# Avokadoen/zig_vulkan

Hardware: AMD Instinct MI355X
Metric: Mrays/s at 1920x1080 on 512^3 brickmap (8^3 bricks, primary + shadow, 1 spp); achieved % of HBM roofline (higher is better)
Workload: dtype f32

## Files before the change

### zig_vulkan_amd/csrc/vrt_api.hip

```cpp
#include <hip/hip_runtime.h>
#include <algorithm>
#include <cstdio>
#include <cstdlib>
#include <cstring>
#include <mutex>
#include <new>
#include <string>
#include <thread>
#include "host_brick_grid.hpp"
#include "vrt_ctx.h"

using namespace vrt_impl;

namespace {
thread_local std::string g_create_error;
}

namespace vrt_impl {

int fail(vrt_ctx *ctx, int code, const std::string &msg) {
    if (ctx) ctx->err = msg;
    else g_create_error = msg;
    return code;
}
// ... 492 lines not shown
        p.split_all = (eligible && waves <= 2u * simds) ? 1u : 0u;
#ifdef VRT_EXP_SPLIT_ALL
        if (c->sched.tile_order == 3u) p.split_all = VRT_EXP_SPLIT_ALL;
#endif
    }
    p.brick_batch = (cfg->kernel_variant >> 24) & 0xFu ? ((cfg->kernel_variant >> 24) & 0xFu) * 4u : 8u;
    p.path_brick_batch = (cfg->kernel_variant >> 24) & 0xFu ? ((cfg->kernel_variant >> 24) & 0xFu) * 4u : 32u;
    p.block_threads = ((vrt::resolve_variant(c->cfg.kernel_variant) & 0xFFu) == vrt::kVariantLinearLds512) ? 512u : 256u;
    {
        auto gcd = [](uint32_t a, uint32_t b) { while (b) { const uint32_t t = a % b; a = b; b = t; } return a; };
        uint32_t st = (uint32_t)((double)sh.owned_tiles * 0.6180339887) | 1u;
        while (sh.owned_tiles > 1u && gcd(st, sh.owned_tiles) != 1u) st += 2u;
        p.tile_stride = sh.owned_tiles > 1u ? st % sh.owned_tiles : 0u;
        if (sh.owned_tiles > 1u && p.tile_stride == 0u) p.tile_stride = 1u;
    }
    p.nbx = nbx;
    p.nby = nby;
    p.nbz = nbz;
    if (c->stream_b) {
        VRT_CREATE_HIP(hipEventRecord(c->ev_upload, c->stream));
        c->upload_seq = 1;
    }
#undef VRT_CREATE_HIP
    note_kernel(c, c->product[2] ? c->product[2] : c->kernel_single1);
    *out = c;
    return VRT_OK;
}

void vrt_destroy(vrt_ctx *ctx) { free_ctx(ctx); }

// ... 169 lines not shown
```

### zig_vulkan_amd/csrc/vrt_internal.h

```cpp
#pragma once
#include <hip/hip_runtime.h>
#include <stddef.h>
#include <stdint.h>
#include "../../include/vrt_hip.h"

namespace vrt {

struct PushConstants {
    vrt_camera_device cam;
    vrt_sun_device sun;
};
static_assert(sizeof(vrt_camera_device) == 96, "Camera.Device is 96 bytes (Camera.zig:183-193)");
static_assert(sizeof(vrt_sun_device) == 32, "Sun.Device is 32 bytes (Sun.zig:13-18)");
static_assert(sizeof(PushConstants) == 128, "push constant range is 128 bytes (ComputePipeline.zig:258-272)");
static_assert(sizeof(vrt_grid_state) == 64, "State.Device is 64 bytes (State.zig:60-79)");
static_assert(sizeof(vrt_material) == 20, "Material is 20 bytes (gpu_types.zig:16-32)");

struct DeviceCounters {
    unsigned long long rays, status_loads, bricks_entered, voxel_steps, hits, grid_steps;
    unsigned long long wave_grid_iters, wave_brick_walks, wave_voxel_iters;
};

struct TileOwnership {
    uint32_t period;
// ... 15 lines not shown
    uint32_t skip_to_box;
    const int *cell_bounds;
    uint32_t status_cells, status_words;
    const uint32_t *start_is_slot;
    uint32_t occupancy_words, count_box;
};
struct BrickArgs {
    const uint32_t *cell_box;
    const uint8_t *status_bytes;
    const vrt_material *materials;
    const uint32_t *brick_status, *brick_index;
    const uint8_t *brick_occupancy;
    const uint32_t *brick_start_index;
    const uint8_t *material_index;
};
static_assert(sizeof(TileArgs) == 64 && sizeof(GridExtra) == 48 && sizeof(BrickArgs) == 64, "16, 12 and 16 dwords: s_load_dwordx16, x8 + x4, x16");

struct TraceParams {
    vrt_grid_state grid;
    PushConstants pcs[8];
    const vrt_material *materials;
    const uint32_t *brick_status;
    const uint32_t *brick_index;
    const uint8_t *brick_occupancy;
    const uint32_t *brick_start_index;
    const uint8_t *material_index;
    uint8_t *target_rgba8;
    float *target_rgba32f;
    DeviceCounters *counters;
    uint32_t width, height;
    uint32_t batch_target_stride;
// ... 43 lines not shown
    uint32_t pool_cus;
    float4 *pool_samples;
    uint32_t pool_walk_k;
    uint32_t pool_brick_thr;
    uint32_t pool_trans_thr;
    uint32_t pool_walk_min;
    uint32_t pool_tiles_x_magic;
    uint32_t wave_groups_bounce;
    uint32_t split_all;
    uint32_t count_box;
    uint32_t skip_to_box;
    uint32_t tile_order;
    alignas(16) TileArgs tile_args;
    GridExtra grid_extra;
    BrickArgs brick_args;
};
static_assert(offsetof(TraceParams, grid) == 0 && offsetof(TraceParams, tile_args) % 16 == 0, "the wide scalar loads' offsets");

constexpr int kMaxBatchFrames = 8;
constexpr int kTileW = 16;
constexpr int kTileH = 16;

enum : uint32_t {
    kVariantDefault = 0,
    kVariantLiteral = 1,
    kVariantBlocked = 2,
    kVariantBlockedLds = 3,
    kVariantLinearWide = 4,
    kVariantLinearAlways = 5,
    kVariantLinearLds = 6,
    kVariantLinearLds512 = 7,
    kVariantLinearAhead = 8,
// ... 9 lines not shown
```

### zig_vulkan_amd/csrc/vrt_trace.hip

```cpp
#include <hip/hip_runtime.h>
#include <cstdlib>
#include "vrt_internal.h"
#include "vrt_kernels.h"

namespace vrt {

template <typename PIX>
__global__ __launch_bounds__(256) void vrt_assemble_kernel(const PIX *__restrict__ gathered, PIX *__restrict__ frame, uint32_t width,
                                                           uint32_t height, uint32_t tiles_x, uint32_t shard_count,
                                                           uint32_t tiles_per_rank ,
                                                           const TileOwnership own, uint32_t frame_src_stride ) {
    gathered += (size_t)blockIdx.z * frame_src_stride;
    frame += (size_t)blockIdx.z * width * height;
    const uint32_t x = blockIdx.x * 64u + (threadIdx.x & 63u);
    const uint32_t y = blockIdx.y * 4u + (threadIdx.x >> 6);
    if (x >= width || y >= height) return;
    const uint32_t t = (y / kTileH) * tiles_x + (x / kTileW);
    uint32_t r, i;
    if (own.period) {
        const uint32_t q = t / own.period, j = t % own.period;
        r = own.owner[j];
        i = q * own.count[r] + own.prefix[j];
    } else {
        r = t % shard_count;
// ... 190 lines not shown
static bool is_path_filter_kernel(KernelFn fn) {
    const KernelEntry *e = kernel_entry_of(fn);
    return e && e->path == 1 && e->filter;
}
const char *kernel_name_of(KernelFn fn) {
    const KernelEntry *e = kernel_entry_of(fn);
    return e ? e->name : "?";
}

static void fill_arg_blocks(TraceParams &q) {
    q.tile_args = TileArgs{q.tile_order, q.wave_groups, q.split_all, q.owned_tiles, q.sched_extra, q.own_period, q.tile_schedule, q.wave_timeline,
                           q.own_count, q.shard_rank, q.shard_count, q.tiles_x, q.width, q.height};
    q.grid_extra = GridExtra{q.scale_pow2, q.inv_grid_scale, q.inv_voxel_scale, q.skip_to_box, q.cell_bounds, q.status_cells, q.status_words, q.start_is_slot,
                             q.occupancy_words, q.count_box};
    q.brick_args = BrickArgs{q.cell_box, q.status_bytes, q.materials, q.brick_status, q.brick_index, q.brick_occupancy, q.brick_start_index, q.material_index};
}

hipError_t launch_trace(KernelFn fn, const TraceParams &params, size_t lds_bytes, hipStream_t stream, uint32_t frames) {
    if (params.owned_tiles == 0 || frames == 0) return hipSuccess;
    TraceParams p = params;
    fill_arg_blocks(p);
    if (const KernelEntry *pe = kernel_entry_of(fn); pe && pe->path == 2) {
        if (!p.work_counter || !p.pool_paths || !p.pool_samples || frames != 1u) return hipErrorInvalidValue;
        hipError_t e = hipMemsetAsync(p.work_counter, 0, kMaxBatchFrames * sizeof(uint32_t), stream);
        if (e != hipSuccess) return e;
        const uint64_t units = (uint64_t)p.owned_tiles * 256u * (uint64_t)(p.pcs[0].cam.samples_per_pixel > 0 ? p.pcs[0].cam.samples_per_pixel : 1);
        const uint32_t per_group = 4u * (64u + pe->pool_slots), fit = (uint32_t)std::min<uint64_t>((units + per_group - 1u) / per_group, 1u << 30);
        const uint32_t hold = p.pool_cus * pe->min_waves;
        const uint32_t groups = fit < hold ? (fit ? fit : 1u) : hold;
        VRT_LAUNCH(fn, dim3(groups, 1), dim3(256), pool_group_lds_bytes(pe->pool_slots, pe->pool_stages), stream, p);
// ... 70 lines not shown
```

### zig_vulkan_amd/csrc/vrt_trace_kernels.h

```cpp
#pragma once
#include <hip/hip_runtime.h>
#include "vrt_internal.h"
#include "vrt_kernels.h"
#include "vrt_math.h"

namespace vrt {

constexpr uint32_t MAT_LAMBERTIAN = 0, MAT_METAL = 1, MAT_DIELECTRIC = 2, MAT_NONE = 3;

struct Ray {
    f3 origin, direction;
    float internal_reflection;
    uint32_t ignore_type_material;
};

struct Hit {
    f3 point, normal;
    float t;
    uint32_t index;
};

template <bool COUNT>
struct Cnt {
    uint32_t rays = 0, status_loads = 0, bricks_entered = 0, voxel_steps = 0, hits = 0, grid_steps = 0;
// ... 740 lines not shown
    BrickArgs a;
    uint32_t occupancy_words;
    uint32_t start_is_slot;
    uint32_t scale_pow2;
    float inv_voxel_scale;
};
template <typename T>
VRT_DI T opaque_uniform(T v) {
    asm volatile("" : "+s"(v));
    return v;
}
template <typename T>
VRT_DI const __attribute__((address_space(1))) T *global_ptr(const T *ptr) {
    return (const __attribute__((address_space(1))) T *)ptr;
}
VRT_DI uint32_t scalar_load_u32(const uint32_t *ptr) {
    uint32_t v;
    asm volatile("s_load_dword %0, %1, 0x0\n\ts_waitcnt lgkmcnt(0)" : "=s"(v) : "s"(ptr));
    return v;
}
typedef __attribute__((ext_vector_type(8))) uint32_t u32x8;
typedef __attribute__((ext_vector_type(16))) uint32_t u32x16;
typedef __attribute__((ext_vector_type(2))) uint32_t u32x2;
VRT_DI unsigned long long kernarg_address() { return (unsigned long long)__builtin_amdgcn_kernarg_segment_ptr(); }
struct DerivedPtrs {
    const int *cell_bounds;
    const uint32_t *start_is_slot;
    uint32_t skip_to_box;
};
VRT_DI TileArgs kernarg_tile_args(DerivedPtrs &dp) {
    u32x16 v;
    u32x2 b, f;
    asm volatile("s_load_dwordx16 %0, %4, %5\n\ts_load_dwordx2 %1, %4, %6\n\ts_load_dwordx2 %2, %4, %7\n\ts_load_dword %3, %4, %8\n\ts_waitcnt lgkmcnt(0)"
                 : "=&s"(v), "=&s"(b), "=&s"(f), "=&s"(dp.skip_to_box)
                 : "s"(kernarg_address()), "n"(offsetof(TraceParams, tile_args)), "n"(offsetof(TraceParams, grid_extra) + offsetof(GridExtra, cell_bounds)),
                   "n"(offsetof(TraceParams, grid_extra) + offsetof(GridExtra, start_is_slot)), "n"(offsetof(TraceParams, grid_extra) + offsetof(GridExtra, skip_to_box)));
    dp.cell_bounds = (const int *)__builtin_bit_cast(unsigned long long, b);
    dp.start_is_slot = (const uint32_t *)__builtin_bit_cast(unsigned long long, f);
    return __builtin_bit_cast(TileArgs, v);
}

struct DerivedWords {
    int bounds[6];
    uint32_t start_is_slot;
};
struct EarlyBox {
    DerivedWords dw;
    float g_min[3], g_scale;
    bool test;
};
VRT_DI vrt_camera_device kernarg_camera_box(uint32_t frame, const DerivedPtrs &dp, EarlyBox &eb) {
    struct Parts { u32x16 a; u32x8 b; } v;
    u32x4 lo, gm;
    u32x2 hi;
    uint32_t flag, sc;
    const unsigned long long ka = kernarg_address();
    const unsigned long long at = ka + offsetof(TraceParams, pcs) + (unsigned long long)frame * sizeof(PushConstants);
    const unsigned long long b = dp.cell_bounds ? (unsigned long long)dp.cell_bounds : ka, f = dp.start_is_slot ? (unsigned long long)dp.start_is_slot : ka;
    asm volatile("s_load_dwordx16 %0, %7, 0x0\n\ts_load_dwordx8 %1, %7, 0x40\n\ts_load_dwordx4 %2, %8, 0x0\n\ts_load_dwordx2 %3, %8, 0x10\n\t"
                 "s_load_dword %4, %9, 0x0\n\ts_load_dwordx4 %5, %10, %11\n\ts_load_dword %6, %10, %12\n\ts_waitcnt lgkmcnt(0)"
                 : "=&s"(v.a), "=&s"(v.b), "=&s"(lo), "=&s"(hi), "=&s"(flag), "=&s"(gm), "=&s"(sc)
                 : "s"(at), "s"(b), "s"(f), "s"(ka), "n"(offsetof(TraceParams, grid) + offsetof(vrt_grid_state, min_point_base_t)),
                   "n"(offsetof(TraceParams, grid) + offsetof(vrt_grid_state, max_point_scale) + 12));
    eb.dw = DerivedWords{{(int)lo.x, (int)lo.y, (int)lo.z, (int)lo.w, (int)hi.x, (int)hi.y}, dp.start_is_slot ? flag : 0u};
    const uint32_t gx = gm.x, gy = gm.y, gz = gm.z;
    eb.g_min[0] = __builtin_bit_cast(float, gx), eb.g_min[1] = __builtin_bit_cast(float, gy), eb.g_min[2] = __builtin_bit_cast(float, gz);
    eb.g_scale = __builtin_bit_cast(float, sc);
    eb.test = dp.cell_bounds != nullptr && dp.skip_to_box != 0u;
    struct Padded { vrt_camera_device cam; uint32_t pad[8]; };
    static_assert(sizeof(Parts) == sizeof(Padded) && offsetof(Parts, b) == 64, "x16 | x8, padded to the alignment of the first");
    return __builtin_bit_cast(Padded, v).cam;
}
VRT_DI vrt_sun_device kernarg_sun(uint32_t frame) {
    u32x8 v;
    const unsigned long long at = kernarg_address() + offsetof(TraceParams, pcs) + (unsigned long long)frame * sizeof(PushConstants) + offsetof(PushConstants, sun);
    asm volatile("s_load_dwordx8 %0, %1, 0x0\n\ts_waitcnt lgkmcnt(0)" : "=&s"(v) : "s"(at));
    return __builtin_bit_cast(vrt_sun_device, v);
}
struct GridArgs {
    vrt_grid_state grid;
    uint32_t scale_pow2;
    float inv_grid_scale, inv_voxel_scale;
    uint32_t skip_to_box;
    const int *cell_bounds;
    uint32_t status_cells, status_words;
    const uint32_t *start_is_slot;
    uint32_t occupancy_words, count_box;
};
static_assert(sizeof(GridArgs) == sizeof(vrt_grid_state) + sizeof(GridExtra) && offsetof(GridArgs, cell_bounds) - 64 == offsetof(GridExtra, cell_bounds) &&
                  offsetof(GridArgs, start_is_slot) - 64 == offsetof(GridExtra, start_is_slot) && offsetof(GridArgs, count_box) - 64 == offsetof(GridExtra, count_box),
              "GridArgs = vrt_grid_state + GridExtra, field for field");
// ... 665 lines not shown
    f3 direction = mk3(0, 0, 0);
    const bool should_refract = transmission_direction(ir, r_in.internal_reflection, r_in.direction, normal, direction);
    if (should_refract && rand_3(hit.point) > 0.5f) {
        scattered = create_ray(hit.point, direction);
        scattered.ignore_type_material = MAT_DIELECTRIC;
        scattered.internal_reflection = ir;
    } else {
        direction = reflect3(r_in.direction, normal);
        scattered = create_ray(hit.point, direction);
    }
    return true;
}

template <int B, bool COUNT, int MODE, bool SCALAR_ENTRY = false, bool REJECT = false, bool KARGS = false>
VRT_DI f3 ray_color_single(const TraceParams &p, const PushConstants &pc, const uint32_t *lds_filter, const Ray &ray, Cnt<COUNT> &c,
                           const EarlyBox *eb = nullptr) {
    f3 color = mk3(0, 0, 0);
    int loop_count = 0;
    Hit hit;
    [[maybe_unused]] vrt_sun_device sun_batch;
    bool sun_enabled = false;
    f3 sun_color = mk3(0, 0, 0);
    if constexpr (!KARGS) sun_enabled = pc.sun.enabled > 0, sun_color = mk3(pc.sun.color[0], pc.sun.color[1], pc.sun.color[2]);
    bool primary_hit;
    if constexpr (KARGS) {
        const f3 inv = mk3(safe_inverse(ray.direction.x), safe_inverse(ray.direction.y), safe_inverse(ray.direction.z));
        const bool miss = eb->test && box_miss(ray.origin, inv, eb->dw.bounds, mk3(eb->g_min[0], eb->g_min[1], eb->g_min[2]), eb->g_scale);
        primary_hit = false;
        if (pc.cam.max_bounce > 0 && __builtin_amdgcn_ballot_w64(!miss) != 0ull) {
            primary_hit = grid_hit<B, COUNT, MODE, false, SCALAR_ENTRY, false, REJECT, KARGS>(p, lds_filter, ray, hit, c, nullptr, &eb->dw, miss);
        }
    } else {
        primary_hit = pc.cam.max_bounce > 0 && grid_hit<B, COUNT, MODE, false, SCALAR_ENTRY, false, REJECT, KARGS>(p, lds_filter, ray, hit, c);
    }
    if constexpr (KARGS) {
        sun_batch = kernarg_sun(blockIdx.y);
        sun_enabled = sun_batch.enabled > 0, sun_color = mk3(sun_batch.color[0], sun_batch.color[1], sun_batch.color[2]);
    }
    const vrt_sun_device &sun = KARGS ? sun_batch : pc.sun;
    if (primary_hit) {
        const uint32_t material = hit.index;
        bool lit = true;
        if (sun_enabled) {
            const f3 sun_position = mk3(sun.position[0], sun.position[1], sun.position[2]);
            const f3 rv = rand_vec3_range(ray.direction.x + ray.direction.z, ray.direction.y + ray.direction.z, -sun.radius,
                                          sun.radius);
            const Ray shadow_ray = create_ray(hit.point, (sun_position + rv) - hit.point);
            Hit shadow_hit;
            lit = !grid_hit<B, COUNT, MODE, false, SCALAR_ENTRY, false, REJECT, KARGS>(p, lds_filter, shadow_ray, shadow_hit, c);
        }
        const vrt_material *m = p.materials + material;
        const uint32_t mtype = m->type;
        const f3 attenuation = mk3(m->albedo_r, m->albedo_g, m->albedo_b);
        loop_count = (mtype <= MAT_DIELECTRIC) ? 1 : 0;
        if (sun_enabled) {
// ... 77 lines not shown
    return (xcd < rem) ? xcd * (q + 1u) + i : rem * (q + 1u) + (xcd - rem) * q + i;
}


VRT_DI uint32_t fresh_lane() {
    uint32_t l;
    asm volatile("v_mbcnt_lo_u32_b32 %0, -1, 0\n\tv_mbcnt_hi_u32_b32 %0, -1, %0" : "=v"(l));
    return l;
}

template <int B, bool COUNT, int MODE, int MIN_WAVES, int SHADE, int BLOCK = 256>
__global__ __launch_bounds__(BLOCK, MIN_WAVES) void vrt_trace_kernel(const TraceParams p) {
    extern __shared__ __attribute__((aligned(16))) uint32_t lds_filter[];
    constexpr bool KARGS = SHADE == 2 && !COUNT && BLOCK == 256 && (MODE == kStatusLinearAlways || MODE == kStatusBytes);
    [[maybe_unused]] TileArgs ta;
    [[maybe_unused]] DerivedPtrs dp;
    if constexpr (KARGS) ta = kernarg_tile_args(dp);
#define VRT_TA(field) (KARGS ? ta.field : p.field)
    if constexpr (MODE == kStatusLinearLds) {
        const uint32_t nvec = (p.status_words + 3u) >> 2;
        const uint4 *src = reinterpret_cast<const uint4 *>(p.brick_status);
        uint4 *dst = reinterpret_cast<uint4 *>(lds_filter);
        for (uint32_t i = threadIdx.x; i < nvec; i += blockDim.x) dst[i] = src[i];
        __syncthreads();
    }
    if constexpr (MODE == kStatusBlockedLds) {
        const uint32_t nwords = (p.nbx * p.nby * p.nbz + 31u) >> 5;
        const uint32_t *src = reinterpret_cast<const uint32_t *>(p.status_blocks + (size_t)p.nbx * p.nby * p.nbz);
        for (uint32_t i = threadIdx.x; i < nwords; i += blockDim.x) lds_filter[i] = src[i];
        __syncthreads();
    }
    const uint32_t unit = VRT_TA(wave_groups) ? (blockIdx.x >> 2) : (BLOCK == 512 ? blockIdx.x * 2u + (threadIdx.x >> 8) : (blockIdx.x >> VRT_TA(split_all)));
    const uint32_t wave = VRT_TA(wave_groups) ? (blockIdx.x & 3u)
// ... 3 lines not shown
    uint32_t split = 0u, half = 0u;
    if (VRT_TA(tile_order) == 5u) {
        const uint32_t *const slot = VRT_TA(tile_schedule) + ((unit & 7u) * ((VRT_TA(owned_tiles) + VRT_TA(sched_extra) + 7u) >> 3) + (unit >> 3));
        const uint32_t entry = KARGS ? scalar_load_u32(slot) : *slot;
        if (entry == 0xFFFFFFFFu) return;
        owned = entry & 0x3FFFFFFFu;
        split = entry >> 31;
        half = (entry >> 30) & 1u;
    } else if (VRT_TA(tile_order) == 6u) {
        owned = unit;
    } else if (VRT_TA(tile_order) == 3u) {
        owned = VRT_TA(owned_tiles) - 1u - unit;
        split = VRT_TA(split_all);
        half = blockIdx.x & ((1u << VRT_TA(split_all)) - 1u);
    } else if (VRT_TA(tile_order) == 4u) {
        owned = (uint32_t)(((unsigned long long)unit * p.tile_stride) % VRT_TA(owned_tiles));
    } else if (VRT_TA(tile_order) == 2u) {
        const uint32_t cm = xcd_slice_index(unit, VRT_TA(owned_tiles));
        const uint32_t col = cm / p.tiles_y, row = cm % p.tiles_y;
        owned = row * VRT_TA(tiles_x) + col;
    } else {
        owned = xcd_slice_index(unit, VRT_TA(owned_tiles));
    }
    const uint32_t tile = VRT_TA(own_period) ? (owned / VRT_TA(own_count)) * VRT_TA(own_period) + p.own_slots[owned % VRT_TA(own_count)] : owned * VRT_TA(shard_count) + VRT_TA(shard_rank);
    const uint32_t tile_x = tile % VRT_TA(tiles_x), tile_y = tile / VRT_TA(tiles_x);
    const uint32_t lane = (SHADE <= 1 && !COUNT) ? fresh_lane() : (threadIdx.x & 63u);
    PushConstants pc_batch;
    [[maybe_unused]] EarlyBox eb;
    if constexpr (KARGS) pc_batch.cam = kernarg_camera_box(blockIdx.y, dp, eb);
    const PushConstants &pc = KARGS ? pc_batch : p.pcs[blockIdx.y];
    const bool dual = SHADE != 2 && !COUNT && split != 0u && !p.packed_rgb && pc.cam.samples_per_pixel == 2;
    const uint32_t pixels = 64u >> split;
    const uint32_t rows = 8u >> split;
    auto place = [&](uint32_t ln, uint32_t &ix, uint32_t &iy) {
        const uint32_t pl = dual ? (ln & (pixels - 1u)) : ln;
        ix = (wave & 1u) * 8u + (pl & 7u);
        iy = (wave >> 1) * 8u + half * rows + ((pl >> 3) & (rows - 1u));
    };
    uint32_t in_x, in_y;
    place(lane, in_x, in_y);
    const uint32_t px = tile_x * kTileW + in_x;
    const uint32_t py = tile_y * kTileH + in_y;

#ifdef VRT_DEV_PROFILE
    if (threadIdx.x < 8) vrt_prof[threadIdx.x] = 0ull;
    __syncthreads();
#endif
    VRT_PROF_BEGIN(tp7);
    const unsigned long long t_begin = (VRT_TA(tile_order) == 5u) ? __builtin_readcyclecounter() : 0ull;
    const unsigned long long wall_begin = VRT_TA(wave_timeline) ? wall_clock64() : 0ull;
    Cnt<COUNT> c;
    const bool inside = (px < VRT_TA(width)) && (py < VRT_TA(height)) && lane < (dual ? 2u * pixels : pixels);
    uint32_t rgba = 0u;
    if (inside) {
        f3 color = mk3(0, 0, 0);
        const int spp = (SHADE == 2) ? 1 : pc.cam.samples_per_pixel;
        const float x0 = (float)px, y0 = (float)py;
        const f3 horizontal = mk3(pc.cam.horizontal[0], pc.cam.horizontal[1], pc.cam.horizontal[2]);
        const f3 vertical = mk3(pc.cam.vertical[0], pc.cam.vertical[1], pc.cam.vertical[2]);
        const f3 llc = mk3(pc.cam.lower_left_corner[0], pc.cam.lower_left_corner[1], pc.cam.lower_left_corner[2]);
        const f3 origin = mk3(pc.cam.origin[0], pc.cam.origin[1], pc.cam.origin[2]);
        if constexpr (SHADE == 2) {
            const float u = (x0 + 0.0f) / (float)(pc.cam.image_width - 1u);
            const float v = (y0 + 0.0f) / (float)(pc.cam.image_height - 1u);
            const f3 ray_dir = fma3(horizontal, splat3(u), llc) + fma3(splat3(v), vertical, -origin);
            color = mk3(0, 0, 0) + ray_color_single<B, COUNT, MODE, false, vrt::reads_cell_box(0, B, COUNT, MODE, SHADE), KARGS>(p, pc, lds_filter, create_ray(origin, ray_dir), c, KARGS ? &eb : nullptr);
        } else {
            const int sample_begin = dual ? (int)(lane >= pixels ? 1u : 0u) : 0, sample_end = dual ? sample_begin + 1 : spp;
            for (int sample_i = sample_begin; sample_i < sample_end; sample_i++) {
                const f3 horizontal = opaque_uniform3(pc.cam.horizontal);
                const f3 vertical = opaque_uniform3(pc.cam.vertical);
                const f3 llc = opaque_uniform3(pc.cam.lower_left_corner);
                const f3 origin = opaque_uniform3(pc.cam.origin);
                const float flag = (sample_i > 0) ? 1.0f : 0.0f;
                float x = x0, y = y0;
                if constexpr ((SHADE <= 1 && !COUNT)) {
                    uint32_t sx, sy;
                    place(fresh_lane(), sx, sy);
                    x = (float)(tile_x * kTileW + sx), y = (float)(tile_y * kTileH + sy);
                }
                const float noise_x = hash_12_jitter(x + (float)sample_i, y, flag);
// ... 9 lines not shown
        if constexpr (SHADE != 2 && !COUNT) {
            if (dual) {
                const uint32_t lane = (SHADE <= 1 && !COUNT) ? fresh_lane() : (threadIdx.x & 63u);
                const int from = (int)((lane + pixels) & 63u);
                const f3 second = mk3(__shfl(color.x, from, 64), __shfl(color.y, from, 64), __shfl(color.z, from, 64));
                color = color + second;
                writer = lane < pixels;
            }
        }
        const float fspp = (float)spp;
        color = mk3(__builtin_sqrtf(color.x / fspp), __builtin_sqrtf(color.y / fspp), __builtin_sqrtf(color.z / fspp));

        size_t o;
        uint32_t ox = in_x, oy = in_y;
        if constexpr ((SHADE <= 1 && !COUNT)) place(fresh_lane(), ox, oy);
        if (p.shard_count > 1u || p.packed_tiles) {
            o = (size_t)owned * (kTileW * kTileH) + oy * kTileW + ox;
        } else {
            o = (size_t)(tile_y * kTileH + oy) * p.width + (tile_x * kTileW + ox);
        }
        rgba = unorm8(color.x) | (unorm8(color.y) << 8) | (unorm8(color.z) << 16) | (255u << 24);
        if (writer) {
            if (!p.packed_rgb) reinterpret_cast<uint32_t *>(p.target_rgba8 + (size_t)blockIdx.y * p.batch_target_stride)[o] = rgba;
            if (p.target_rgba32f) {
                reinterpret_cast<float4 *>(p.target_rgba32f)[o] = make_float4(color.x, color.y, color.z, 1.0f);
            }
        }
    }
    if (p.packed_rgb) {
        const uint32_t lane = (SHADE <= 1 && !COUNT) ? fresh_lane() : (threadIdx.x & 63u);
        uint32_t in_x, in_y;
        place(lane, in_x, in_y);
        const uint32_t k = lane & 7u;
        const uint32_t first = k + (k >= 3u ? 1u : 0u);
        const int src = (int)((lane & ~7u) + first);
        const uint32_t lo = (uint32_t)__shfl((int)rgba, src, 64), hi = (uint32_t)__shfl((int)rgba, src + 1, 64);
        const uint32_t m = k % 3u;
        const uint32_t dword = (m == 0u) ? ((lo & 0xFFFFFFu) | (hi << 24)) : ((m == 1u) ? (((lo >> 8) & 0xFFFFu) | (hi << 16)) : (((lo >> 16) & 0xFFu) | (hi << 8)));
        if (k < 6u && lane < (64u >> split))
            reinterpret_cast<uint32_t *>(p.target_rgba8 + (size_t)blockIdx.y * p.batch_target_stride)[(size_t)owned * 192u + in_y * 12u + (in_x >> 3) * 6u + k] = dword;
    }
    const uint32_t lane_end = (SHADE <= 1 && !COUNT) ? fresh_lane() : lane;
#ifdef VRT_DEV_PROFILE
    VRT_PROF_END(7, tp7);
    __syncthreads();
    if (p.wave_timeline && threadIdx.x < 8) p.wave_timeline[(size_t)blockIdx.x * 8 + threadIdx.x] = vrt_prof[threadIdx.x];
#else
    if (p.wave_timeline && lane_end == 0) {
        const size_t w_id = (size_t)blockIdx.x * (blockDim.x >> 6) + (((SHADE <= 1 && !COUNT) && BLOCK != 512) ? (p.wave_groups ? 0u : wave) : (threadIdx.x >> 6));
        p.wave_timeline[2 * w_id] = wall_begin;
        p.wave_timeline[2 * w_id + 1] = wall_clock64();
    }
#endif
    if (p.tile_order == 5u) {
        const unsigned long long dt = __builtin_readcyclecounter() - t_begin;
        if (lane_end == 0) p.tile_cost[((size_t)half * p.owned_tiles + owned) * 4u + wave] = (uint32_t)(dt >> 6);
    }
    if constexpr (COUNT) {
        unsigned long long v[9] = {c.rays, c.status_loads, c.bricks_entered, c.voxel_steps, c.hits, c.grid_steps,
                                   c.wave_grid_iters, c.wave_brick_walks, c.wave_voxel_iters};
#pragma unroll
        for (int k = 0; k < 9; k++) {
            unsigned long long s = v[k];
            for (int off = 32; off > 0; off >>= 1) s += __shfl_down(s, off, 64);
            v[k] = s;
        }
        if (lane_end == 0) {
            atomicAdd(&p.counters->rays, v[0]);
            atomicAdd(&p.counters->status_loads, v[1]);
            atomicAdd(&p.counters->bricks_entered, v[2]);
            atomicAdd(&p.counters->voxel_steps, v[3]);
            atomicAdd(&p.counters->hits, v[4]);
            atomicAdd(&p.counters->grid_steps, v[5]);
            atomicAdd(&p.counters->wave_grid_iters, v[6]);
            atomicAdd(&p.counters->wave_brick_walks, v[7]);
            atomicAdd(&p.counters->wave_voxel_iters, v[8]);
        }
    }
}

#undef VRT_TA

}
```

Baseline: 39620.

## Batch kernarg scalar loads, replace tile divisions with magic reciprocals, hoist trace

```diff
diff --git a/zig_vulkan_amd/csrc/vrt_api.hip b/zig_vulkan_amd/csrc/vrt_api.hip
--- a/zig_vulkan_amd/csrc/vrt_api.hip
+++ b/zig_vulkan_amd/csrc/vrt_api.hip
@@ -530,6 +530,12 @@
         p.tile_stride = sh.owned_tiles > 1u ? st % sh.owned_tiles : 0u;
         if (sh.owned_tiles > 1u && p.tile_stride == 0u) p.tile_stride = 1u;
     }
+    if (!vrt::magic_exact_below(sh.tiles_x * sh.tiles_y + 64u, sh.tiles_x) || !vrt::magic_exact_below(sh.tiles_x * sh.tiles_y + 64u, sh.tiles_y) ||
+        (p.own_period && !vrt::magic_exact_below(sh.owned_tiles + 1u, p.own_count)) ||
+        (p.tile_order == 4u && sh.owned_tiles > 1u && !vrt::magic_mulmod_exact_below(sh.owned_tiles, p.tile_stride, sh.owned_tiles))) {
+        free_ctx(c);
+        return fail(nullptr, VRT_E_OUT_OF_RANGE, "the tile index does not divide exactly by the multiply-high reciprocal (vrt_magic_div.h)");
+    }
     p.nbx = nbx;
     p.nby = nby;
     p.nbz = nbz;
diff --git a/zig_vulkan_amd/csrc/vrt_internal.h b/zig_vulkan_amd/csrc/vrt_internal.h
--- a/zig_vulkan_amd/csrc/vrt_internal.h
+++ b/zig_vulkan_amd/csrc/vrt_internal.h
@@ -3,6 +3,8 @@
 #include <stddef.h>
 #include <stdint.h>
 #include "../../include/vrt_hip.h"
+#define VRT_MAGIC_FN __host__ __device__ inline
+#include "vrt_magic_div.h"
 
 namespace vrt {
 
@@ -53,7 +55,15 @@
     const uint32_t *brick_start_index;
     const uint8_t *material_index;
 };
-static_assert(sizeof(TileArgs) == 64 && sizeof(GridExtra) == 48 && sizeof(BrickArgs) == 64, "16, 12 and 16 dwords: s_load_dwordx16, x8 + x4, x16");
+struct StoreArgs {
+    const vrt_material *materials;
+    uint8_t *target_rgba8;
+    float *target_rgba32f;
+    uint32_t *tile_cost;
+    uint32_t shard_count, packed_tiles, packed_rgb, width, batch_target_stride, owned_tiles, tile_order, timeline;
+};
+static_assert(sizeof(TileArgs) == 64 && sizeof(GridExtra) == 48 && sizeof(BrickArgs) == 64 && sizeof(StoreArgs) == 64,
+              "16, 12, 16 and 16 dwords: s_load_dwordx16, x8 + x4, x16, x16");
 
 struct TraceParams {
     vrt_grid_state grid;
@@ -127,8 +137,12 @@
     alignas(16) TileArgs tile_args;
     GridExtra grid_extra;
     BrickArgs brick_args;
+    StoreArgs store_args;
+    alignas(16) uint32_t tile_magic[4];
 };
-static_assert(offsetof(TraceParams, grid) == 0 && offsetof(TraceParams, tile_args) % 16 == 0, "the wide scalar loads' offsets");
+static_assert(offsetof(TraceParams, grid) == 0 && offsetof(TraceParams, tile_args) % 16 == 0 && offsetof(TraceParams, store_args) % 16 == 0 &&
+                  offsetof(TraceParams, tile_magic) % 16 == 0 && offsetof(TraceParams, own_slots) % 4 == 0,
+              "the wide scalar loads' offsets");
 
 constexpr int kMaxBatchFrames = 8;
 constexpr int kTileW = 16;
diff --git a/zig_vulkan_amd/csrc/vrt_magic_div.h b/zig_vulkan_amd/csrc/vrt_magic_div.h
--- /dev/null
+++ b/zig_vulkan_amd/csrc/vrt_magic_div.h
@@ -0,0 +1,49 @@
+#pragma once
+#include <stdint.h>
+
+#ifndef VRT_MAGIC_FN
+#define VRT_MAGIC_FN inline
+#endif
+
+namespace vrt {
+
+struct MagicQuotRem {
+    uint32_t quot, rem;
+};
+
+VRT_MAGIC_FN uint32_t magic_of(uint32_t d) {
+    return d == 0u ? 0u : (d == 1u ? 0xFFFFFFFFu : (uint32_t)((1ull << 32) / d));
+}
+
+VRT_MAGIC_FN MagicQuotRem magic_divmod(uint32_t n, uint32_t d, uint32_t magic) {
+    uint32_t q = (uint32_t)(((unsigned long long)n * magic) >> 32);
+    uint32_t r = n - q * d;
+    if (r >= d) q += 1u, r -= d;
+    return MagicQuotRem{q, r};
+}
+
+VRT_MAGIC_FN uint32_t magic_mulmod(uint32_t a, uint32_t b, uint32_t d, uint32_t magic) {
+    uint32_t r = magic_divmod(((a >> 16) & 0xFFu) * b, d, magic).rem;
+    r = magic_divmod(r * 256u + ((a >> 8) & 0xFFu) * b, d, magic).rem;
+    return magic_divmod(r * 256u + (a & 0xFFu) * b, d, magic).rem;
+}
+VRT_MAGIC_FN bool magic_mulmod_exact_below(uint32_t count, uint32_t b, uint32_t d) {
+    if (d == 0u) return true;
+    if (b >= d || d >= (1u << 23) || count > (1u << 24)) return false;
+    const uint32_t magic = magic_of(d);
+    for (uint32_t a = 0; a < count; a++)
+        if (magic_mulmod(a, b, d, magic) != (uint32_t)(((unsigned long long)a * b) % d)) return false;
+    return true;
+}
+
+VRT_MAGIC_FN bool magic_exact_below(uint32_t count, uint32_t d) {
+    if (d == 0u) return true;
+    const uint32_t magic = magic_of(d);
+    for (uint32_t n = 0; n < count; n++) {
+        const MagicQuotRem m = magic_divmod(n, d, magic);
+        if (m.quot != n / d || m.rem != n % d) return false;
+    }
+    return true;
+}
+
+}
diff --git a/zig_vulkan_amd/csrc/vrt_trace.hip b/zig_vulkan_amd/csrc/vrt_trace.hip
--- a/zig_vulkan_amd/csrc/vrt_trace.hip
+++ b/zig_vulkan_amd/csrc/vrt_trace.hip
@@ -228,6 +228,12 @@
     q.grid_extra = GridExtra{q.scale_pow2, q.inv_grid_scale, q.inv_voxel_scale, q.skip_to_box, q.cell_bounds, q.status_cells, q.status_words, q.start_is_slot,
                              q.occupancy_words, q.count_box};
     q.brick_args = BrickArgs{q.cell_box, q.status_bytes, q.materials, q.brick_status, q.brick_index, q.brick_occupancy, q.brick_start_index, q.material_index};
+    q.store_args = StoreArgs{q.materials, q.target_rgba8, q.target_rgba32f, q.tile_cost, q.shard_count, q.packed_tiles, q.packed_rgb, q.width,
+                             q.batch_target_stride, q.owned_tiles, q.tile_order, q.wave_timeline ? 1u : 0u};
+    q.tile_magic[0] = magic_of(q.tiles_x);
+    q.tile_magic[1] = q.own_period ? magic_of(q.own_count) : 0u;
+    q.tile_magic[2] = magic_of(q.tiles_y);
+    q.tile_magic[3] = magic_of(q.owned_tiles);
 }
 
 hipError_t launch_trace(KernelFn fn, const TraceParams &params, size_t lds_bytes, hipStream_t stream, uint32_t frames) {
diff --git a/zig_vulkan_amd/csrc/vrt_trace_kernels.h b/zig_vulkan_amd/csrc/vrt_trace_kernels.h
--- a/zig_vulkan_amd/csrc/vrt_trace_kernels.h
+++ b/zig_vulkan_amd/csrc/vrt_trace_kernels.h
@@ -1,5 +1,6 @@
 #pragma once
 #include <hip/hip_runtime.h>
+#include <type_traits>
 #include "vrt_internal.h"
 #include "vrt_kernels.h"
 #include "vrt_math.h"
@@ -778,6 +779,10 @@
 VRT_DI const __attribute__((address_space(1))) T *global_ptr(const T *ptr) {
     return (const __attribute__((address_space(1))) T *)ptr;
 }
+template <typename T>
+VRT_DI void store_to(T *ptr, const T &v) {
+    *(__attribute__((address_space(1))) T *)ptr = v;
+}
 VRT_DI uint32_t scalar_load_u32(const uint32_t *ptr) {
     uint32_t v;
     asm volatile("s_load_dword %0, %1, 0x0\n\ts_waitcnt lgkmcnt(0)" : "=s"(v) : "s"(ptr));
@@ -787,20 +792,50 @@
 typedef __attribute__((ext_vector_type(16))) uint32_t u32x16;
 typedef __attribute__((ext_vector_type(2))) uint32_t u32x2;
 VRT_DI unsigned long long kernarg_address() { return (unsigned long long)__builtin_amdgcn_kernarg_segment_ptr(); }
+VRT_DI unsigned long long kernarg_u64(uint32_t offset) {
+    u32x2 v;
+    asm volatile("s_load_dwordx2 %0, %1, 0x0\n\ts_waitcnt lgkmcnt(0)" : "=&s"(v) : "s"(kernarg_address() + offset));
+    return __builtin_bit_cast(unsigned long long, v);
+}
 struct DerivedPtrs {
     const int *cell_bounds;
     const uint32_t *start_is_slot;
     uint32_t skip_to_box;
 };
-VRT_DI TileArgs kernarg_tile_args(DerivedPtrs &dp) {
+struct FirstBatch {
+    DerivedPtrs dp;
+    vrt_camera_device cam;
+    float g_min[3], g_scale;
+    uint32_t tiles_x_magic, own_count_magic, tiles_y_magic, owned_tiles_magic;
+    unsigned long long own_slots[2];
+};
+VRT_DI TileArgs kernarg_first_batch(uint32_t frame, FirstBatch &fb) {
+    struct Parts { u32x16 a; u32x8 b; } cam;
     u32x16 v;
+    u32x4 gm, slots, magic;
     u32x2 b, f;
-    asm volatile("s_load_dwordx16 %0, %4, %5\n\ts_load_dwordx2 %1, %4, %6\n\ts_load_dwordx2 %2, %4, %7\n\ts_load_dword %3, %4, %8\n\ts_waitcnt lgkmcnt(0)"
-                 : "=&s"(v), "=&s"(b), "=&s"(f), "=&s"(dp.skip_to_box)
-                 : "s"(kernarg_address()), "n"(offsetof(TraceParams, tile_args)), "n"(offsetof(TraceParams, grid_extra) + offsetof(GridExtra, cell_bounds)),
-                   "n"(offsetof(TraceParams, grid_extra) + offsetof(GridExtra, start_is_slot)), "n"(offsetof(TraceParams, grid_extra) + offsetof(GridExtra, skip_to_box)));
-    dp.cell_bounds = (const int *)__builtin_bit_cast(unsigned long long, b);
-    dp.start_is_slot = (const uint32_t *)__builtin_bit_cast(unsigned long long, f);
+    uint32_t sc;
+    const unsigned long long ka = kernarg_address();
+    const unsigned long long at = ka + offsetof(TraceParams, pcs) + (unsigned long long)frame * sizeof(PushConstants);
+    asm volatile("s_load_dwordx16 %0, %10, %12\n\ts_load_dwordx2 %1, %10, %13\n\ts_load_dwordx2 %2, %10, %14\n\ts_load_dword %3, %10, %15\n\t"
+                 "s_load_dwordx4 %4, %10, %16\n\ts_load_dwordx4 %5, %10, %17\n\ts_load_dwordx16 %6, %11, 0x0\n\ts_load_dwordx8 %7, %11, 0x40\n\t"
+                 "s_load_dwordx4 %8, %10, %18\n\ts_load_dword %9, %10, %19\n\ts_waitcnt lgkmcnt(0)"
+                 : "=&s"(v), "=&s"(b), "=&s"(f), "=&s"(fb.dp.skip_to_box), "=&s"(magic), "=&s"(slots), "=&s"(cam.a), "=&s"(cam.b), "=&s"(gm), "=&s"(sc)
+                 : "s"(ka), "s"(at), "n"(offsetof(TraceParams, tile_args)), "n"(offsetof(TraceParams, grid_extra) + offsetof(GridExtra, cell_bounds)),
+                   "n"(offsetof(TraceParams, grid_extra) + offsetof(GridExtra, start_is_slot)), "n"(offsetof(TraceParams, grid_extra) + offsetof(GridExtra, skip_to_box)),
+                   "n"(offsetof(TraceParams, tile_magic)), "n"(offsetof(TraceParams, own_slots)),
+                   "n"(offsetof(TraceParams, grid) + offsetof(vrt_grid_state, min_point_base_t)),
+                   "n"(offsetof(TraceParams, grid) + offsetof(vrt_grid_state, max_point_scale) + 12));
+    fb.dp.cell_bounds = (const int *)__builtin_bit_cast(unsigned long long, b);
+    fb.dp.start_is_slot = (const uint32_t *)__builtin_bit_cast(unsigned long long, f);
+    fb.tiles_x_magic = magic.x, fb.own_count_magic = magic.y, fb.tiles_y_magic = magic.z, fb.owned_tiles_magic = magic.w;
+    fb.own_slots[0] = (unsigned long long)slots.x | ((unsigned long long)slots.y << 32), fb.own_slots[1] = (unsigned long long)slots.z | ((unsigned long long)slots.w << 32);
+    const uint32_t gx = gm.x, gy = gm.y, gz = gm.z;
+    fb.g_min[0] = __builtin_bit_cast(float, gx), fb.g_min[1] = __builtin_bit_cast(float, gy), fb.g_min[2] = __builtin_bit_cast(float, gz);
+    fb.g_scale = __builtin_bit_cast(float, sc);
+    struct Padded { vrt_camera_device cam; uint32_t pad[8]; };
+    static_assert(sizeof(Parts) == sizeof(Padded) && offsetof(Parts, b) == 64, "x16 | x8, padded to the alignment of the first");
+    fb.cam = __builtin_bit_cast(Padded, cam).cam;
     return __builtin_bit_cast(TileArgs, v);
 }
 
@@ -813,32 +848,41 @@
     float g_min[3], g_scale;
     bool test;
 };
-VRT_DI vrt_camera_device kernarg_camera_box(uint32_t frame, const DerivedPtrs &dp, EarlyBox &eb) {
-    struct Parts { u32x16 a; u32x8 b; } v;
-    u32x4 lo, gm;
+VRT_DI void scalar_early_box(const FirstBatch &fb, EarlyBox &eb) {
+    u32x4 lo;
     u32x2 hi;
-    uint32_t flag, sc;
+    uint32_t flag;
+    const DerivedPtrs &dp = fb.dp;
     const unsigned long long ka = kernarg_address();
-    const unsigned long long at = ka + offsetof(TraceParams, pcs) + (unsigned long long)frame * sizeof(PushConstants);
     const unsigned long long b = dp.cell_bounds ? (unsigned long long)dp.cell_bounds : ka, f = dp.start_is_slot ? (unsigned long long)dp.start_is_slot : ka;
-    asm volatile("s_load_dwordx16 %0, %7, 0x0\n\ts_load_dwordx8 %1, %7, 0x40\n\ts_load_dwordx4 %2, %8, 0x0\n\ts_load_dwordx2 %3, %8, 0x10\n\t"
-                 "s_load_dword %4, %9, 0x0\n\ts_load_dwordx4 %5, %10, %11\n\ts_load_dword %6, %10, %12\n\ts_waitcnt lgkmcnt(0)"
-                 : "=&s"(v.a), "=&s"(v.b), "=&s"(lo), "=&s"(hi), "=&s"(flag), "=&s"(gm), "=&s"(sc)
-                 : "s"(at), "s"(b), "s"(f), "s"(ka), "n"(offsetof(TraceParams, grid) + offsetof(vrt_grid_state, min_point_base_t)),
-                   "n"(offsetof(TraceParams, grid) + offsetof(vrt_grid_state, max_point_scale) + 12));
+    asm volatile("s_load_dwordx4 %0, %3, 0x0\n\ts_load_dwordx2 %1, %3, 0x10\n\ts_load_dword %2, %4, 0x0\n\ts_waitcnt lgkmcnt(0)"
+                 : "=&s"(lo), "=&s"(hi), "=&s"(flag)
+                 : "s"(b), "s"(f));
     eb.dw = DerivedWords{{(int)lo.x, (int)lo.y, (int)lo.z, (int)lo.w, (int)hi.x, (int)hi.y}, dp.start_is_slot ? flag : 0u};
-    const uint32_t gx = gm.x, gy = gm.y, gz = gm.z;
-    eb.g_min[0] = __builtin_bit_cast(float, gx), eb.g_min[1] = __builtin_bit_cast(float, gy), eb.g_min[2] = __builtin_bit_cast(float, gz);
-    eb.g_scale = __builtin_bit_cast(float, sc);
+    eb.g_min[0] = fb.g_min[0], eb.g_min[1] = fb.g_min[1], eb.g_min[2] = fb.g_min[2];
+    eb.g_scale = fb.g_scale;
     eb.test = dp.cell_bounds != nullptr && dp.skip_to_box != 0u;
-    struct Padded { vrt_camera_device cam; uint32_t pad[8]; };
-    static_assert(sizeof(Parts) == sizeof(Padded) && offsetof(Parts, b) == 64, "x16 | x8, padded to the alignment of the first");
-    return __builtin_bit_cast(Padded, v).cam;
 }
 VRT_DI vrt_sun_device kernarg_sun(uint32_t frame) {
     u32x8 v;
     const unsigned long long at = kernarg_address() + offsetof(TraceParams, pcs) + (unsigned long long)frame * sizeof(PushConstants) + offsetof(PushConstants, sun);
     asm volatile("s_load_dwordx8 %0, %1, 0x0\n\ts_waitcnt lgkmcnt(0)" : "=&s"(v) : "s"(at));
+    return __builtin_bit_cast(vrt_sun_device, v);
+}
+VRT_DI StoreArgs kernarg_store_args() {
+    u32x16 v;
+    asm volatile("s_load_dwordx16 %0, %1, %2\n\ts_waitcnt lgkmcnt(0)" : "=&s"(v) : "s"(kernarg_address()), "n"(offsetof(TraceParams, store_args)));
+    return __builtin_bit_cast(StoreArgs, v);
+}
+VRT_DI vrt_sun_device kernarg_sun_store_args(uint32_t frame, StoreArgs &st) {
+    u32x8 v;
+    u32x16 w;
+    const unsigned long long ka = kernarg_address();
+    const unsigned long long at = ka + offsetof(TraceParams, pcs) + (unsigned long long)frame * sizeof(PushConstants) + offsetof(PushConstants, sun);
+    asm volatile("s_load_dwordx8 %0, %2, 0x0\n\ts_load_dwordx16 %1, %3, %4\n\ts_waitcnt lgkmcnt(0)"
+                 : "=&s"(v), "=&s"(w)
+                 : "s"(at), "s"(ka), "n"(offsetof(TraceParams, store_args)));
+    st = __builtin_bit_cast(StoreArgs, w);
     return __builtin_bit_cast(vrt_sun_device, v);
 }
 struct GridArgs {
@@ -1534,7 +1578,7 @@
 
 template <int B, bool COUNT, int MODE, bool SCALAR_ENTRY = false, bool REJECT = false, bool KARGS = false>
 VRT_DI f3 ray_color_single(const TraceParams &p, const PushConstants &pc, const uint32_t *lds_filter, const Ray &ray, Cnt<COUNT> &c,
-                           const EarlyBox *eb = nullptr) {
+                           const EarlyBox *eb = nullptr, StoreArgs *st = nullptr, bool outside = false) {
     f3 color = mk3(0, 0, 0);
     int loop_count = 0;
     Hit hit;
@@ -1545,7 +1589,7 @@
     bool primary_hit;
     if constexpr (KARGS) {
         const f3 inv = mk3(safe_inverse(ray.direction.x), safe_inverse(ray.direction.y), safe_inverse(ray.direction.z));
-        const bool miss = eb->test && box_miss(ray.origin, inv, eb->dw.bounds, mk3(eb->g_min[0], eb->g_min[1], eb->g_min[2]), eb->g_scale);
+        const bool miss = outside || (eb->test && box_miss(ray.origin, inv, eb->dw.bounds, mk3(eb->g_min[0], eb->g_min[1], eb->g_min[2]), eb->g_scale));
         primary_hit = false;
         if (pc.cam.max_bounce > 0 && __builtin_amdgcn_ballot_w64(!miss) != 0ull) {
             primary_hit = grid_hit<B, COUNT, MODE, false, SCALAR_ENTRY, false, REJECT, KARGS>(p, lds_filter, ray, hit, c, nullptr, &eb->dw, miss);
@@ -1554,11 +1598,36 @@
         primary_hit = pc.cam.max_bounce > 0 && grid_hit<B, COUNT, MODE, false, SCALAR_ENTRY, false, REJECT, KARGS>(p, lds_filter, ray, hit, c);
     }
     if constexpr (KARGS) {
-        sun_batch = kernarg_sun(blockIdx.y);
-        sun_enabled = sun_batch.enabled > 0, sun_color = mk3(sun_batch.color[0], sun_batch.color[1], sun_batch.color[2]);
-    }
-    const vrt_sun_device &sun = KARGS ? sun_batch : pc.sun;
-    if (primary_hit) {
+        if (__builtin_amdgcn_ballot_w64(primary_hit) != 0ull) {
+            sun_batch = kernarg_sun(blockIdx.y);
+            sun_enabled = sun_batch.enabled > 0, sun_color = mk3(sun_batch.color[0], sun_batch.color[1], sun_batch.color[2]);
+            bool lit = true;
+            if (primary_hit && sun_enabled) {
+                const f3 sun_position = mk3(sun_batch.position[0], sun_batch.position[1], sun_batch.position[2]);
+                const f3 rv = rand_vec3_range(ray.direction.x + ray.direction.z, ray.direction.y + ray.direction.z, -sun_batch.radius,
+                                              sun_batch.radius);
+                const Ray shadow_ray = create_ray(hit.point, (sun_position + rv) - hit.point);
+                Hit shadow_hit;
+                lit = !grid_hit<B, COUNT, MODE, false, SCALAR_ENTRY, false, REJECT, KARGS>(p, lds_filter, shadow_ray, shadow_hit, c);
+            }
+            *st = kernarg_store_args();
+            if (primary_hit) {
+                const auto *m = global_ptr(st->materials) + hit.index;
+                const uint32_t mtype = m->type;
+                const f3 attenuation = mk3(m->albedo_r, m->albedo_g, m->albedo_b);
+                loop_count = (mtype <= MAT_DIELECTRIC) ? 1 : 0;
+                if (sun_enabled) {
+                    if (lit) color = color + attenuation * sun_color;
+                } else {
+                    color = color + attenuation;
+                }
+            }
+        } else {
+            sun_batch = kernarg_sun_store_args(blockIdx.y, *st);
+            sun_enabled = sun_batch.enabled > 0, sun_color = mk3(sun_batch.color[0], sun_batch.color[1], sun_batch.color[2]);
+        }
+    } else if (primary_hit) {
+        const vrt_sun_device &sun = pc.sun;
         const uint32_t material = hit.index;
         bool lit = true;
         if (sun_enabled) {
@@ -1666,9 +1735,11 @@
     extern __shared__ __attribute__((aligned(16))) uint32_t lds_filter[];
     constexpr bool KARGS = SHADE == 2 && !COUNT && BLOCK == 256 && (MODE == kStatusLinearAlways || MODE == kStatusBytes);
     [[maybe_unused]] TileArgs ta;
-    [[maybe_unused]] DerivedPtrs dp;
-    if constexpr (KARGS) ta = kernarg_tile_args(dp);
+    [[maybe_unused]] FirstBatch fb;
+    [[maybe_unused]] StoreArgs st;
+    if constexpr (KARGS) ta = kernarg_first_batch(blockIdx.y, fb);
 #define VRT_TA(field) (KARGS ? ta.field : p.field)
+#define VRT_ST(field) (KARGS ? st.field : p.field)
     if constexpr (MODE == kStatusLinearLds) {
         const uint32_t nvec = (p.status_words + 3u) >> 2;
         const uint4 *src = reinterpret_cast<const uint4 *>(p.brick_status);
@@ -1702,20 +1773,39 @@
         split = VRT_TA(split_all);
         half = blockIdx.x & ((1u << VRT_TA(split_all)) - 1u);
     } else if (VRT_TA(tile_order) == 4u) {
-        owned = (uint32_t)(((unsigned long long)unit * p.tile_stride) % VRT_TA(owned_tiles));
+        if constexpr (KARGS) owned = magic_mulmod(unit, p.tile_stride, ta.owned_tiles, fb.owned_tiles_magic);
+        else owned = (uint32_t)(((unsigned long long)unit * p.tile_stride) % VRT_TA(owned_tiles));
     } else if (VRT_TA(tile_order) == 2u) {
         const uint32_t cm = xcd_slice_index(unit, VRT_TA(owned_tiles));
-        const uint32_t col = cm / p.tiles_y, row = cm % p.tiles_y;
-        owned = row * VRT_TA(tiles_x) + col;
+        if constexpr (KARGS) {
+            const MagicQuotRem cr = magic_divmod(cm, p.tiles_y, fb.tiles_y_magic);
+            owned = cr.rem * ta.tiles_x + cr.quot;
+        } else {
+            const uint32_t col = cm / p.tiles_y, row = cm % p.tiles_y;
+            owned = row * VRT_TA(tiles_x) + col;
+        }
     } else {
         owned = xcd_slice_index(unit, VRT_TA(owned_tiles));
     }
-    const uint32_t tile = VRT_TA(own_period) ? (owned / VRT_TA(own_count)) * VRT_TA(own_period) + p.own_slots[owned % VRT_TA(own_count)] : owned * VRT_TA(shard_count) + VRT_TA(shard_rank);
-    const uint32_t tile_x = tile % VRT_TA(tiles_x), tile_y = tile / VRT_TA(tiles_x);
+    uint32_t tile, tile_x, tile_y;
+    if constexpr (KARGS) {
+        if (ta.own_period) {
+            const MagicQuotRem o = magic_divmod(owned, ta.own_count, fb.own_count_magic);
+            const uint32_t slot = (uint32_t)((o.rem < 8u ? fb.own_slots[0] : fb.own_slots[1]) >> ((o.rem & 7u) * 8u)) & 0xFFu;
+            tile = o.quot * ta.own_period + slot;
+        } else {
+            tile = owned * ta.shard_count + ta.shard_rank;
+        }
+        const MagicQuotRem t = magic_divmod(tile, ta.tiles_x, fb.tiles_x_magic);
+        tile_x = t.rem, tile_y = t.quot;
+    } else {
+        tile = VRT_TA(own_period) ? (owned / VRT_TA(own_count)) * VRT_TA(own_period) + p.own_slots[owned % VRT_TA(own_count)] : owned * VRT_TA(shard_count) + VRT_TA(shard_rank);
+        tile_x = tile % VRT_TA(tiles_x), tile_y = tile / VRT_TA(tiles_x);
+    }
     const uint32_t lane = (SHADE <= 1 && !COUNT) ? fresh_lane() : (threadIdx.x & 63u);
     PushConstants pc_batch;
     [[maybe_unused]] EarlyBox eb;
-    if constexpr (KARGS) pc_batch.cam = kernarg_camera_box(blockIdx.y, dp, eb);
+    if constexpr (KARGS) pc_batch.cam = fb.cam, scalar_early_box(fb, eb);
     const PushConstants &pc = KARGS ? pc_batch : p.pcs[blockIdx.y];
     const bool dual = SHADE != 2 && !COUNT && split != 0u && !p.packed_rgb && pc.cam.samples_per_pixel == 2;
     const uint32_t pixels = 64u >> split;
@@ -1740,6 +1830,18 @@
     Cnt<COUNT> c;
     const bool inside = (px < VRT_TA(width)) && (py < VRT_TA(height)) && lane < (dual ? 2u * pixels : pixels);
     uint32_t rgba = 0u;
+    struct Nothing {};
+    [[maybe_unused]] typename std::conditional<KARGS, f3, Nothing>::type traced;
+    if constexpr (KARGS) {
+        const f3 horizontal = mk3(pc.cam.horizontal[0], pc.cam.horizontal[1], pc.cam.horizontal[2]);
+        const f3 vertical = mk3(pc.cam.vertical[0], pc.cam.vertical[1], pc.cam.vertical[2]);
+        const f3 llc = mk3(pc.cam.lower_left_corner[0], pc.cam.lower_left_corner[1], pc.cam.lower_left_corner[2]);
+        const f3 origin = mk3(pc.cam.origin[0], pc.cam.origin[1], pc.cam.origin[2]);
+        const float u = ((float)px + 0.0f) / (float)(pc.cam.image_width - 1u);
+        const float v = ((float)py + 0.0f) / (float)(pc.cam.image_height - 1u);
+        const f3 ray_dir = fma3(horizontal, splat3(u), llc) + fma3(splat3(v), vertical, -origin);
+        traced = ray_color_single<B, COUNT, MODE, false, vrt::reads_cell_box(0, B, COUNT, MODE, SHADE), KARGS>(p, pc, lds_filter, create_ray(origin, ray_dir), c, &eb, &st, !inside);
+    }
     if (inside) {
         f3 color = mk3(0, 0, 0);
         const int spp = (SHADE == 2) ? 1 : pc.cam.samples_per_pixel;
@@ -1752,7 +1854,8 @@
             const float u = (x0 + 0.0f) / (float)(pc.cam.image_width - 1u);
             const float v = (y0 + 0.0f) / (float)(pc.cam.image_height - 1u);
             const f3 ray_dir = fma3(horizontal, splat3(u), llc) + fma3(splat3(v), vertical, -origin);
-            color = mk3(0, 0, 0) + ray_color_single<B, COUNT, MODE, false, vrt::reads_cell_box(0, B, COUNT, MODE, SHADE), KARGS>(p, pc, lds_filter, create_ray(origin, ray_dir), c, KARGS ? &eb : nullptr);
+            if constexpr (KARGS) color = mk3(0, 0, 0) + traced;
+            else color = mk3(0, 0, 0) + ray_color_single<B, COUNT, MODE, false, vrt::reads_cell_box(0, B, COUNT, MODE, SHADE), KARGS>(p, pc, lds_filter, create_ray(origin, ray_dir), c);
         } else {
             const int sample_begin = dual ? (int)(lane >= pixels ? 1u : 0u) : 0, sample_end = dual ? sample_begin + 1 : spp;
             for (int sample_i = sample_begin; sample_i < sample_end; sample_i++) {
@@ -1792,20 +1895,26 @@
         size_t o;
         uint32_t ox = in_x, oy = in_y;
         if constexpr ((SHADE <= 1 && !COUNT)) place(fresh_lane(), ox, oy);
-        if (p.shard_count > 1u || p.packed_tiles) {
+        if (VRT_ST(shard_count) > 1u || VRT_ST(packed_tiles)) {
             o = (size_t)owned * (kTileW * kTileH) + oy * kTileW + ox;
         } else {
-            o = (size_t)(tile_y * kTileH + oy) * p.width + (tile_x * kTileW + ox);
+            o = (size_t)(tile_y * kTileH + oy) * VRT_ST(width) + (tile_x * kTileW + ox);
         }
         rgba = unorm8(color.x) | (unorm8(color.y) << 8) | (unorm8(color.z) << 16) | (255u << 24);
         if (writer) {
-            if (!p.packed_rgb) reinterpret_cast<uint32_t *>(p.target_rgba8 + (size_t)blockIdx.y * p.batch_target_stride)[o] = rgba;
-            if (p.target_rgba32f) {
-                reinterpret_cast<float4 *>(p.target_rgba32f)[o] = make_float4(color.x, color.y, color.z, 1.0f);
-            }
-        }
-    }
-    if (p.packed_rgb) {
+            if constexpr (KARGS) {
+                typedef __attribute__((ext_vector_type(4))) float f32x4;
+                if (!st.packed_rgb) store_to(&reinterpret_cast<uint32_t *>(st.target_rgba8 + (size_t)blockIdx.y * st.batch_target_stride)[o], rgba);
+                if (st.target_rgba32f) store_to(&reinterpret_cast<f32x4 *>(st.target_rgba32f)[o], f32x4{color.x, color.y, color.z, 1.0f});
+            } else {
+                if (!p.packed_rgb) reinterpret_cast<uint32_t *>(p.target_rgba8 + (size_t)blockIdx.y * p.batch_target_stride)[o] = rgba;
+                if (p.target_rgba32f) {
+                    reinterpret_cast<float4 *>(p.target_rgba32f)[o] = make_float4(color.x, color.y, color.z, 1.0f);
+                }
+            }
+        }
+    }
+    if (VRT_ST(packed_rgb)) {
         const uint32_t lane = (SHADE <= 1 && !COUNT) ? fresh_lane() : (threadIdx.x & 63u);
         uint32_t in_x, in_y;
         place(lane, in_x, in_y);
@@ -1816,7 +1925,10 @@
         const uint32_t m = k % 3u;
         const uint32_t dword = (m == 0u) ? ((lo & 0xFFFFFFu) | (hi << 24)) : ((m == 1u) ? (((lo >> 8) & 0xFFFFu) | (hi << 16)) : (((lo >> 16) & 0xFFu) | (hi << 8)));
         if (k < 6u && lane < (64u >> split))
-            reinterpret_cast<uint32_t *>(p.target_rgba8 + (size_t)blockIdx.y * p.batch_target_stride)[(size_t)owned * 192u + in_y * 12u + (in_x >> 3) * 6u + k] = dword;
+        {
+            if constexpr (KARGS) store_to(&reinterpret_cast<uint32_t *>(st.target_rgba8 + (size_t)blockIdx.y * st.batch_target_stride)[(size_t)owned * 192u + in_y * 12u + (in_x >> 3) * 6u + k], dword);
+            else reinterpret_cast<uint32_t *>(p.target_rgba8 + (size_t)blockIdx.y * p.batch_target_stride)[(size_t)owned * 192u + in_y * 12u + (in_x >> 3) * 6u + k] = dword;
+        }
     }
     const uint32_t lane_end = (SHADE <= 1 && !COUNT) ? fresh_lane() : lane;
 #ifdef VRT_DEV_PROFILE
@@ -1824,15 +1936,26 @@
     __syncthreads();
     if (p.wave_timeline && threadIdx.x < 8) p.wave_timeline[(size_t)blockIdx.x * 8 + threadIdx.x] = vrt_prof[threadIdx.x];
 #else
-    if (p.wave_timeline && lane_end == 0) {
+    if constexpr (KARGS) {
+        if (st.timeline != 0u && lane_end == 0) {
+            unsigned long long *const timeline = (unsigned long long *)kernarg_u64(offsetof(TraceParams, wave_timeline));
+            const size_t w_id = (size_t)blockIdx.x * (blockDim.x >> 6) + (threadIdx.x >> 6);
+            store_to(&timeline[2 * w_id], wall_begin);
+            store_to(&timeline[2 * w_id + 1], (unsigned long long)wall_clock64());
+        }
+    } else if (p.wave_timeline && lane_end == 0) {
         const size_t w_id = (size_t)blockIdx.x * (blockDim.x >> 6) + (((SHADE <= 1 && !COUNT) && BLOCK != 512) ? (p.wave_groups ? 0u : wave) : (threadIdx.x >> 6));
         p.wave_timeline[2 * w_id] = wall_begin;
         p.wave_timeline[2 * w_id + 1] = wall_clock64();
     }
 #endif
-    if (p.tile_order == 5u) {
+    if (VRT_ST(tile_order) == 5u) {
         const unsigned long long dt = __builtin_readcyclecounter() - t_begin;
-        if (lane_end == 0) p.tile_cost[((size_t)half * p.owned_tiles + owned) * 4u + wave] = (uint32_t)(dt >> 6);
+        if constexpr (KARGS) {
+            if (lane_end == 0) store_to(&st.tile_cost[((size_t)half * st.owned_tiles + owned) * 4u + wave], (uint32_t)(dt >> 6));
+        } else {
+            if (lane_end == 0) p.tile_cost[((size_t)half * p.owned_tiles + owned) * 4u + wave] = (uint32_t)(dt >> 6);
+        }
     }
     if constexpr (COUNT) {
         unsigned long long v[9] = {c.rays, c.status_loads, c.bricks_entered, c.voxel_steps, c.hits, c.grid_steps,
@@ -1858,5 +1981,6 @@
 }
 
 #undef VRT_TA
-
-}
+#undef VRT_ST
+
+}
```

Result: no change. 39540 (-0.2%).
